# xuhuifan/FFVD

Measured on AMD Instinct MI355X. Metric: ELBO iters/sec (T=4096, M=512, x_dim=4, S=32), higher is better.
Workload: dtype f64; 1 GPU; c2: synthetic T=4096 x_dim=4 C=1 M=512 S=32 SquaredExponential collapsed-U, seed 20230209; chains_per_gpu=32, dims_per_gpu=4, arithmetic=fp64 throughout

## Files before the change

### ffvd_amd/csrc/kernels.hip

```cpp
#include "kernels.h"
#include "dev_common.h"
#define FFVD_STEP_TRACE_OWNER
#include "step_bodies.h"
#if defined(FFVD_STEP_TRACE)
extern "C" int ffvd_debug_step_spans(unsigned long long *out) {
    return (int)hipMemcpyFromSymbol(out, HIP_SYMBOL(ffvd::step_span), sizeof(unsigned long long) * 64 * 4 * 2);
}
extern "C" int ffvd_debug_step_trace(long long *out) {
    return (int)hipMemcpyFromSymbol(out, HIP_SYMBOL(ffvd::step_trace_buf), sizeof(long long) * 4096 * 8);
}
#endif
#include <type_traits>
#include <cstdlib>

namespace ffvd {

__device__ __forceinline__ double block_sum_256(double v, double *scratch ) {
    const int tid = threadIdx.x;
    scratch[tid] = v;
    __syncthreads();
    for (int s = 128; s > 0; s >>= 1) {
        if (tid < s) scratch[tid] += scratch[tid + s];
        __syncthreads();
    }
// ... 182 lines not shown
                        const double *log_Q, double yn_over_batch, double *H, size_t h_stride, int brow) {
    hipLaunchKernelGGL(brow_finish_kernel, dim3((Mp + 255) / 256, nb), dim3(256), 0, stream, gpart, nblk, Mp, Dl, d_begin, b0, log_Q,
                       yn_over_batch, H, h_stride, brow);
}
template <bool NT>
static void launch_kfu_build_nt(hipStream_t stream, const ProjectArgs &a) {
    dim3 grid(a.Tp / 64, a.Mp / 64, a.nb);
    if (a.P <= 8) {
        const int nq = (a.P + 1) / 2;
        if (a.kind == 0) {
            if (nq <= 2) hipLaunchKernelGGL((kfu_build_kernel<0, 2, NT>), grid, dim3(256), 0, stream, a);
            else if (nq == 3) hipLaunchKernelGGL((kfu_build_kernel<0, 3, NT>), grid, dim3(256), 0, stream, a);
            else hipLaunchKernelGGL((kfu_build_kernel<0, 4, NT>), grid, dim3(256), 0, stream, a);
        } else hipLaunchKernelGGL((kfu_build_kernel<1, 4, NT>), grid, dim3(256), 0, stream, a);
    } else {
        if (a.kind == 0) hipLaunchKernelGGL((kfu_build_kernel<0, 0, NT>), grid, dim3(256), 0, stream, a);
        else hipLaunchKernelGGL((kfu_build_kernel<1, 0, NT>), grid, dim3(256), 0, stream, a);
    }
}
template <int KIND, int NQ, int MW>
__global__ __launch_bounds__(256) void kfu_build_t_kernel(ProjectArgs a, int ldt) {
    kfu_build_t_body<KIND, NQ, MW>(a, ldt, blockIdx.x, blockIdx.y, blockIdx.z);
}
void launch_kfu_build_t(hipStream_t stream, const ProjectArgs &a, int ldt) {
    constexpr int MW = 4;
    dim3 grid(a.Tp / 64, a.Mp / (4 * MW), a.nb);
    if (a.P <= 8) {
        const int nq = (a.P + 1) / 2;
        if (a.kind == 0) {
            if (nq <= 2) hipLaunchKernelGGL((kfu_build_t_kernel<0, 2, MW>), grid, dim3(256), 0, stream, a, ldt);
            else if (nq == 3) hipLaunchKernelGGL((kfu_build_t_kernel<0, 3, MW>), grid, dim3(256), 0, stream, a, ldt);
            else hipLaunchKernelGGL((kfu_build_t_kernel<0, 4, MW>), grid, dim3(256), 0, stream, a, ldt);
        } else hipLaunchKernelGGL((kfu_build_t_kernel<1, 4, MW>), grid, dim3(256), 0, stream, a, ldt);
    } else {
        if (a.kind == 0) hipLaunchKernelGGL((kfu_build_t_kernel<0, 0, MW>), grid, dim3(256), 0, stream, a, ldt);
        else hipLaunchKernelGGL((kfu_build_t_kernel<1, 0, MW>), grid, dim3(256), 0, stream, a, ldt);
    }
}
void launch_kfu_build(hipStream_t stream, const ProjectArgs &a) {
    const bool nt = (size_t)a.nb * a.Tp * a.Mp * sizeof(double) >= ((size_t)1 << 30);
    if (nt) launch_kfu_build_nt<true>(stream, a);
    else launch_kfu_build_nt<false>(stream, a);
}

__global__ __launch_bounds__(256) void kernel_matrix_kernel(int kind, const double *X, int N, const double *X2, int N2,
                                                            int P, double logvar, const double *loglen, double jitter,
                                                            int same, double *out) {
    const size_t idx = (size_t)blockIdx.x * 256 + threadIdx.x;
    if (idx >= (size_t)N * N2) return;
    const int i = (int)(idx / N2), j = (int)(idx % N2);
    const double var = exp(logvar);
    const double *xi = X + (size_t)i * P, *zj = X2 + (size_t)j * P;
    double v;
    if (kind == 0) {
        double dot = 0.0, xx = 0.0, zz = 0.0;
        for (int p = 0; p < P; ++p) {
            double l = exp(loglen[p]);
            double a = xi[p] / l, b = zj[p] / l;
            dot += a * b; xx += a * a; zz += b * b;
        }
        v = kernel_value<0>(dot, xx, zz, var);
    } else {
        double dot = 0.0;
        for (int p = 0; p < P; ++p) dot += (xi[p] * var) * zj[p];
        v = dot;
    }
    if (same && i == j) v += jitter;
    out[idx] = v;
}
void launch_kernel_matrix(hipStream_t stream, int kind, const double *X, int N, const double *X2, int N2, int P,
                          double logvar, const double *loglen_dev, double jitter, int same, double *out) {
    size_t n = (size_t)N * N2;
    if (n == 0) return;
    hipLaunchKernelGGL(kernel_matrix_kernel, dim3((unsigned)((n + 255) / 256)), dim3(256), 0, stream, kind, X, N, X2,
                       N2, P, logvar, loglen_dev, jitter, same, out);
}
__global__ void kernel_diag_kernel(int kind, const double *X, int N, int P, double logvar, double *out) {
    int i = blockIdx.x * blockDim.x + threadIdx.x;
    if (i >= N) return;
    const double var = exp(logvar);
    if (kind == 0) { out[i] = var; return; }
    double s = 0.0;
    for (int p = 0; p < P; ++p) { double x = X[(size_t)i * P + p]; s += (x * x) * var; }
    out[i] = s;
}
void launch_kernel_diag(hipStream_t stream, int kind, const double *X, int N, int P, double logvar, double *out) {
    if (N == 0) return;
    hipLaunchKernelGGL(kernel_diag_kernel, dim3((N + 255) / 256), dim3(256), 0, stream, kind, X, N, P, logvar, out);
}

#ifdef FFVD_DF_TRACE
__device__ long long df_trace_buf[64 * 64];
__device__ long long gram_trace_buf[128 * 10 * 4];
#endif

constexpr int LR_LD = NB + 2;
constexpr int DV_LD = 17;
template <bool PIPE>
__device__ __forceinline__ int chol64_1w(double (&a)[NB], double (*Lr)[LR_LD], double *invd, const int lane) {
    int bad = 0;
    if (!PIPE) {
#pragma unroll
        for (int j = 0; j < NB; ++j) {
            double s0 = a[j], s1 = 0.0;
            if (j >= 2) wave_lds_sync();
#pragma unroll
            for (int i = 0; i + 1 < j - 1 + (j & 1); i += 2) {
                const double2 lj = *reinterpret_cast<const double2 *>(&Lr[j][i]);
                s0 -= a[i] * lj.x;
                s1 -= a[i + 1] * lj.y;
            }
            if (j >= 2 && !(j & 1)) s0 -= a[j - 2] * Lr[j][j - 2];
            if (j >= 1) s1 -= a[j - 1] * readlane_f64(a[j - 1], j);
            const double v = s0 + s1;
            const double ajj = readlane_f64(v, j);
            if (!(ajj > 0.0) && bad == 0) bad = j + 1;
            double piv, y;
            pivot_sqrt(ajj, piv, y);
            a[j] = v * y;
            Lr[lane][j] = a[j];
            if (lane == 0) invd[j] = y;
        }
        return bad;
    }
    double nxt = 0.0;
#pragma unroll
    for (int j = 0; j < NB; ++j) {
        double v = a[j] - nxt;
        if (j >= 2) v -= a[j - 2] * readlane_f64(a[j - 2], j);
        if (j >= 1) v -= a[j - 1] * readlane_f64(a[j - 1], j);
        const double ajj = readlane_f64(v, j);
        if (!(ajj > 0.0) && bad == 0) bad = j + 1;
        double piv, y;
        pivot_sqrt(ajj, piv, y);
        if (j + 1 < NB) {
            if (j >= 2) wave_lds_sync();
            double q0 = 0.0, q1 = 0.0, q2 = 0.0, q3 = 0.0;
#pragma unroll
            for (int i = 0; i + 1 <= j - 2; i += 2) {
                const double2 l2 = *reinterpret_cast<const double2 *>(&Lr[j + 1][i]);
                if (i & 2) { q2 += a[i] * l2.x; q3 += a[i + 1] * l2.y; }
                else { q0 += a[i] * l2.x; q1 += a[i + 1] * l2.y; }
            }
            if (j >= 2 && !(j & 1)) q0 += a[j - 2] * Lr[j + 1][j - 2];
            nxt = (q0 + q1) + (q2 + q3);
        }
        a[j] = v * y;
        Lr[lane][j] = a[j];
        if (lane == 0) invd[j] = y;
    }
    return bad;
}

__device__ __forceinline__ int chol64_mfma_4w(double (*Ts)[NB + 1], double (*Lr)[LR_LD], double (*Sc)[16][DV_LD], double *dinv_b) {
    const int lane = threadIdx.x & 63, lr = lane & 15, lk = lane >> 4;
    const int wave = __builtin_amdgcn_readfirstlane((int)(threadIdx.x >> 6));
    if (threadIdx.x < 256) Sc[3][threadIdx.x >> 4][threadIdx.x & 15] = ((threadIdx.x >> 4) == (threadIdx.x & 15)) ? 1.0 : 0.0;
    __syncthreads();
    int bad = 0;
#pragma unroll
    for (int s = 0; s < 4; ++s) {
        const int s0 = 16 * s;
        if (s > 0) {
            const int i = s + wave;
            if (i < 4) {
                const int i0 = 16 * i;
                d4 acc = (d4){0.0, 0.0, 0.0, 0.0}, acc1 = acc;
                for (int k = 0; k < s; ++k)
#pragma unroll
                    for (int t = 0; t < 4; ++t) {
                        const double av = Lr[i0 + lr][16 * k + 4 * t + lk], bv = Lr[s0 + lr][16 * k + 4 * t + lk];
                        if (t & 1) acc1 = mfma_f64(av, bv, acc1);
                        else acc = mfma_f64(av, bv, acc);
                    }
#pragma unroll
                for (int r = 0; r < 4; ++r) Sc[wave][lk + 4 * r][lr] = Ts[i0 + lk + 4 * r][s0 + lr] - (acc[r] + acc1[r]);
            }
            __syncthreads();
        }
        if (wave == 0 || (s == 0 && wave == 1)) {
            __builtin_amdgcn_s_setprio(3);
            int tl;
            if (wave == 0) tl = (lk == 0) ? 0 : (lk == 1) ? -1 : ((s + lk - 1 < 4) ? lk - 1 : -2);
            else tl = (lk == 1) ? 3 : -2;
            const double *src;
            if (tl == -1) src = &Sc[3][lr][0];
            else if (s == 0) src = &Ts[16 * (tl > 0 ? tl : 0) + lr][0];
            else src = &Sc[tl > 0 ? tl : 0][lr][0];
            double a[16];
#pragma unroll
            for (int c = 0; c < 16; ++c) a[c] = src[c];
#pragma unroll
            for (int j = 0; j < 16; ++j) {
                const double ajj = readlane_f64(a[j], j);
                double piv, y;
                pivot_sqrt(ajj, piv, y);
                a[j] *= y;
#pragma unroll
                for (int c = j + 1; c < 16; ++c) a[c] = fma(-a[j], readlane_f64(a[j], c), a[c]);
            }
            double diag = a[0];
#pragma unroll
            for (int c = 1; c < 16; ++c) diag = (lr == c) ? a[c] : diag;
            if (tl >= 0) {
                double *base = &Lr[s0 + 16 * tl + lr][s0];
#pragma unroll
                for (int c = 0; c < 16; ++c) base[c] = (tl > 0 || c <= lr) ? a[c] : 0.0;
            } else if (tl == -1) {
#pragma unroll
                for (int c = 0; c < 16; ++c) dinv_b[(s0 + c) * 16 + lr] = a[c];
            }
            if (wave == 0) {
                const unsigned long long m = __ballot((lane < 16) & !(diag > 0.0));
                if (m && !bad) bad = s0 + (int)__builtin_ctzll(m) + 1;
            }
            __builtin_amdgcn_s_setprio(0);
        }
        __syncthreads();
    }
    return bad;
}

template <bool PIPE>
__device__ __forceinline__ void diag_block_finish(double (*Ts)[NB + 1], double (*Lr)[LR_LD], double *invd, double *S, int n,
                                                   int k0, int32_t *info_b, double *dinv_b, double (*Sc)[16][DV_LD] = nullptr) {
    const int tid = threadIdx.x, lane = tid & 63;
    const int w = __builtin_amdgcn_readfirstlane(tid >> 6);
    if (Sc) {
        const int bad = chol64_mfma_4w(Ts, Lr, Sc, dinv_b);
        if (w == 0 && bad && lane == 0 && *info_b == 0) *info_b = k0 + bad;
        for (int r = tid >> 6; r < NB; r += 4)
            if (lane <= r) S[(size_t)(k0 + r) * n + k0 + lane] = Lr[r][lane];
        return;
    }
    if (w == 0) {
        double a[NB];
#pragma unroll
        for (int c = 0; c < NB; ++c) a[c] = Ts[lane][c];
        __builtin_amdgcn_s_setprio(3);
        const int bad = chol64_1w<PIPE>(a, Lr, invd, lane);
        __builtin_amdgcn_s_setprio(0);
        if (bad && lane == 0 && *info_b == 0) *info_b = k0 + bad;
    }
    __syncthreads();
    for (int r = tid >> 6; r < NB; r += 4)
        if (lane <= r) S[(size_t)(k0 + r) * n + k0 + lane] = Lr[r][lane];
    if (lane < 16) {
        const int o = 16 * w;
        double x[16];
#pragma unroll
        for (int r = 0; r < 16; ++r) {
            double acc = (lane == r) ? 1.0 : 0.0;
#pragma unroll
            for (int i = 0; i < r; ++i) acc -= Lr[o + r][o + i] * x[i];
            x[r] = acc * invd[o + r];
        }
#pragma unroll
        for (int r = 0; r < 16; ++r) dinv_b[(w * 16 + r) * 16 + lane] = x[r];
    }
}

__global__ __launch_bounds__(256) void potrf_diag_kernel(double *A, int n, int k, size_t slab_stride, int32_t *info,
                                                         double *dinv) {
    __shared__ double Ts[NB][NB + 1];
    __shared__ double Lr[NB][LR_LD];
    __shared__ double invd[NB];
    const int b = blockIdx.x, tid = threadIdx.x;
    double *S = A + (size_t)b * slab_stride;
    const int k0 = k * NB;
    for (int r = tid >> 6; r < NB; r += 4) Ts[r][tid & 63] = S[(size_t)(k0 + r) * n + k0 + (tid & 63)];
    __syncthreads();
    diag_block_finish<true>(Ts, Lr, invd, S, n, k0, info + b, dinv + (size_t)b * DINV_STRIDE);
}

__device__ __forceinline__ int extra_block(int e, int nlive, int nid) { return (e < nlive) ? e : nid + (e - nlive); }
__device__ __forceinline__ int chunk_row0(int chunk, int k, int nmain, int n, int nlive, int nid) {
    return (chunk < nmain) ? (k + 1 + chunk) * NB : n + extra_block(chunk - nmain, nlive, nid) * NB;
}

constexpr int TR_LD = NB + 2;

__global__ __launch_bounds__(256) void potrf_panel_kernel(double *A, int n, int k, int nmain, size_t slab_stride,
                                                          int nlive, int nid, const double *dinv) {
    __shared__ double Ls[NB][TR_LD];
    __shared__ double Dv[4][16][DV_LD];
    const int b = blockIdx.y, tid = threadIdx.x, lane = tid & 63, lr = lane & 15, lk = lane >> 4;
    const int w = __builtin_amdgcn_readfirstlane(tid >> 6);
    double *S = A + (size_t)b * slab_stride;
    const int k0 = k * NB;
    const int row0 = chunk_row0(blockIdx.x, k, nmain, n, nlive, nid);
    double *Rl = S + (size_t)(row0 + 16 * w + lr) * n + k0 + lk;
    d4 Rt[4];
#pragma unroll
    for (int s4 = 0; s4 < 4; ++s4)
#pragma unroll
        for (int r = 0; r < 4; ++r) Rt[s4][r] = Rl[16 * s4 + 4 * r];
#pragma unroll
    for (int i = 0; i < 8; ++i) {
        const int r = (tid >> 5) + 8 * i, c2 = 2 * (tid & 31);
        const double2 v = *reinterpret_cast<const double2 *>(S + (size_t)(k0 + r) * n + k0 + c2);
        Ls[r][c2] = (c2 <= r) ? -v.x : 0.0;
        Ls[r][c2 + 1] = (c2 + 1 <= r) ? -v.y : 0.0;
    }
    {
        const double *dv = dinv + (size_t)b * DINV_STRIDE;
#pragma unroll
        for (int i = 0; i < 4; ++i) {
            const int e = tid + 256 * i;
            Dv[e >> 8][(e >> 4) & 15][e & 15] = dv[e];
        }
    }
    __syncthreads();
#pragma unroll
    for (int s4 = 0; s4 < 4; ++s4) {
        d4 x = (d4){0.0, 0.0, 0.0, 0.0};
#pragma unroll
        for (int ks = 0; ks < 4; ++ks) x = mfma_f64(Dv[s4][lr][4 * ks + lk], Rt[s4][ks], x);
        d4 res = Rt[s4];
#pragma unroll
        for (int ks = 0; ks < 4; ++ks) res = mfma_f64(Ls[16 * s4 + lr][16 * s4 + 4 * ks + lk], x[ks], res);
#pragma unroll
        for (int ks = 0; ks < 4; ++ks) x = mfma_f64(Dv[s4][lr][4 * ks + lk], res[ks], x);
        Rt[s4] = x;
#pragma unroll
        for (int t = s4 + 1; t < 4; ++t)
#pragma unroll
            for (int ks = 0; ks < 4; ++ks) Rt[t] = mfma_f64(Ls[16 * t + lr][16 * s4 + 4 * ks + lk], x[ks], Rt[t]);
    }
#pragma unroll
    for (int s4 = 0; s4 < 4; ++s4)
#pragma unroll
        for (int r = 0; r < 4; ++r) Rl[16 * s4 + 4 * r] = Rt[s4][r];
}

template <bool PIPE>
__global__ __launch_bounds__(256) void potrf_trail_kernel(double *A, int n, int k, int nmain_tiles, int n1,
                                                          size_t slab_stride, int32_t *info, int nlive, int nid,
                                                          double *dinv) {
    constexpr int HLD = 34;
    __shared__ double sm[2 * NB * HLD];
    __shared__ double invd[NB];
    static_assert(2 * NB * HLD >= NB * LR_LD, "the staging buffer must hold the factor tile");
    double *Pi_h = sm, *Pj_h = sm + NB * HLD;
    const int b = blockIdx.y;
    const int tile = blockIdx.x;
    double *S = A + (size_t)b * slab_stride;
    const int k0 = k * NB;
    int rowblk0, colblk;
    if (tile < nmain_tiles) {
        int i = 0;
        while ((i + 1) * (i + 2) / 2 <= tile) ++i;
        int j = tile - i * (i + 1) / 2;
        rowblk0 = (k + 1 + i) * NB;
        colblk = (k + 1 + j) * NB;
    } else {
        int t = tile - nmain_tiles;
        int e = t / n1, j = t % n1;
        rowblk0 = n + extra_block(e, nlive, nid) * NB;
        colblk = (k + 1 + j) * NB;
    }
    const int tid = threadIdx.x, lane = tid & 63, lr = lane & 15, lk = lane >> 4;
    const int wave = __builtin_amdgcn_readfirstlane(tid >> 6);
    const int qr = wave >> 1, qc = wave & 1;
    const bool same = (rowblk0 == colblk);
    const double *Pi = S + (size_t)rowblk0 * n + k0;
    const double *Pj = S + (size_t)colblk * n + k0;
    const int sr = tid >> 4, sc = 2 * (tid & 15);
    double2 vi[2][4], vj[2][4];
#pragma unroll
    for (int h = 0; h < 2; ++h)
#pragma unroll
        for (int i = 0; i < 4; ++i) {
            vi[h][i] = *reinterpret_cast<const double2 *>(Pi + (size_t)(sr + 16 * i) * n + 32 * h + sc);
            if (!same) vj[h][i] = *reinterpret_cast<const double2 *>(Pj + (size_t)(sr + 16 * i) * n + 32 * h + sc);
        }
    const double *Bh = same ? Pi_h : Pj_h;
    double *Ct = S + (size_t)rowblk0 * n + colblk;
    d4 cold[2][2];
#pragma unroll
    for (int x = 0; x < 2; ++x)
#pragma unroll
        for (int y = 0; y < 2; ++y)
#pragma unroll
            for (int q = 0; q < 4; ++q)
                cold[x][y][q] = Ct[(size_t)(qr * 32 + 16 * x + lk + 4 * q) * n + qc * 32 + 16 * y + lr];
// ... 171 lines not shown
#pragma unroll
    for (int s4 = 0; s4 < 4; ++s4) {
        d4 x = (d4){0.0, 0.0, 0.0, 0.0};
#pragma unroll
        for (int ks = 0; ks < 4; ++ks) x = mfma_f64(Dv[s4][lr][4 * ks + lk], Rt[s4][ks], x);
        d4 res = Rt[s4];
#pragma unroll
        for (int ks = 0; ks < 4; ++ks) res = mfma_f64(Ls[16 * s4 + lr][16 * s4 + 4 * ks + lk], x[ks], res);
#pragma unroll
        for (int ks = 0; ks < 4; ++ks) x = mfma_f64(Dv[s4][lr][4 * ks + lk], res[ks], x);
        Rt[s4] = x;
#pragma unroll
        for (int t = s4 + 1; t < 4; ++t)
#pragma unroll
            for (int ks = 0; ks < 4; ++ks) Rt[t] = mfma_f64(Ls[16 * t + lr][16 * s4 + 4 * ks + lk], x[ks], Rt[t]);
    }
    double *Rl = S + (size_t)(row0 + 16 * wave + lr) * n + j0 + lk;
#pragma unroll
    for (int s4 = 0; s4 < 4; ++s4)
#pragma unroll
        for (int r = 0; r < 4; ++r) Rl[16 * s4 + 4 * r] = Rt[s4][r];
    if (!look) return;
#pragma unroll
    for (int s4 = 0; s4 < 4; ++s4)
#pragma unroll
        for (int r = 0; r < 4; ++r) Xs[16 * wave + lr][16 * s4 + 4 * r + lk] = Rt[s4][r];
    __syncthreads();
    if (do_d) {
#pragma unroll 4
        for (int ks = 0; ks < NB / 4; ++ks) {
            double ax[2], bx[2];
#pragma unroll
            for (int x = 0; x < 2; ++x) {
                ax[x] = Xs[qr * 32 + 16 * x + lr][4 * ks + lk];
                bx[x] = Xs[qc * 32 + 16 * x + lr][4 * ks + lk];
            }
#pragma unroll
            for (int x = 0; x < 2; ++x)
#pragma unroll
                for (int y = 0; y < 2; ++y) acc_d[x][y] = mfma_f64(ax[x], bx[y], acc_d[x][y]);
        }
    }
    double (*Ts)[NB + 1] = reinterpret_cast<double(*)[NB + 1]>(sm1);
    double (*Lr)[LR_LD] = reinterpret_cast<double(*)[LR_LD]>(sm1);
#pragma unroll
    for (int x = 0; x < 2; ++x)
#pragma unroll
        for (int y = 0; y < 2; ++y)
#pragma unroll
            for (int q = 0; q < 4; ++q)
                Ts[qr * 32 + 16 * x + lk + 4 * q][qc * 32 + 16 * y + lr] = cold_d[x][y][q] - acc_d[x][y][q];
    __syncthreads();
    diag_block_finish<PIPE>(Ts, Lr, invd, S, n, j0 + NB, info + b, dinv + (size_t)b * DINV_STRIDE + ((j + 1) & 1) * (DINV_STRIDE / 2));
}

__global__ __launch_bounds__(256) void diag_inv_kernel(const double *A, int n, int j, size_t slab_stride, double *dinv) {
    __shared__ double Lr[NB][NB + 1];
    const int b = blockIdx.x, tid = threadIdx.x, lane = tid & 63;
    const int w = __builtin_amdgcn_readfirstlane(tid >> 6);
    const double *S = A + (size_t)b * slab_stride;
    const int j0 = j * NB;
    for (int r = tid >> 6; r < NB; r += 4) Lr[r][lane] = S[(size_t)(j0 + r) * n + j0 + lane];
    __syncthreads();
    if (lane < 16) {
        const int o = 16 * w;
        double x[16];
#pragma unroll
        for (int r = 0; r < 16; ++r) {
            double acc = (lane == r) ? 1.0 : 0.0;
#pragma unroll
            for (int i = 0; i < r; ++i) acc -= Lr[o + r][o + i] * x[i];
            x[r] = acc / Lr[o + r][o + r];
        }
        double *dv = dinv + (size_t)b * DINV_STRIDE + (j & 1) * (DINV_STRIDE / 2);
#pragma unroll
        for (int r = 0; r < 16; ++r) dv[(w * 16 + r) * 16 + lane] = x[r];
    }
}

void launch_trsm_ext(hipStream_t stream, double *A, int n, int extra_rows, int batch, size_t slab_stride, double *dinv) {
    const int nb = n / NB, ntail = extra_rows / NB;
    if (ntail == 0) return;
    const int groups = (batch + 7) / 8;
    for (int j = 0; j < nb; ++j) {
        hipLaunchKernelGGL(diag_inv_kernel, dim3(batch), dim3(256), 0, stream, A, n, j, slab_stride, dinv);
        hipLaunchKernelGGL(potrf_ll_kernel<false>, dim3(groups * 8 * ntail), dim3(256), 0, stream, A, n, j, 0, ntail,
                           slab_stride, (int32_t *)nullptr, 0, 0, batch, dinv);
    }
}

constexpr int DF_PS = 64;
static_assert(DF_PS == 64, "launch_kuu_build zeroes 64 progress words per matrix");
constexpr int DF_DINV = 4 * 16 * 16;
constexpr long long DF_SPIN_TICKS = 100000000LL;

struct DfArgs {
    double *A;
    int n, nb, next, nid, batch, G;
    size_t slab_stride;
    int32_t *info;
    double *dinv;
    int *prog;
    int *abort_w;
    double *xt;
    size_t xt_stride;
    int vec_tail;
    double *kinv;
    size_t kinv_stride;
    int defer_ext;
    int kinv_help;
    int fine;
    const double *lt;
    size_t lt_stride;
    int lt_dl;
};

#ifdef FFVD_DF_TRACE
#define DF_STAMP(row, slot) do { if ((row) >= 0 && threadIdx.x == 0) df_trace_buf[(row) * 64 + (slot)] = wall_clock64(); } while (0)
extern "C" int ffvd_debug_df_trace(long long *out) {
    return (int)hipMemcpyFromSymbol(out, HIP_SYMBOL(df_trace_buf), sizeof(long long) * 64 * 64);
}
extern "C" int ffvd_debug_gram_trace(long long *out) {
    return (int)hipMemcpyFromSymbol(out, HIP_SYMBOL(gram_trace_buf), sizeof(long long) * 128 * 10 * 4);
}
#else
#define DF_STAMP(row, slot) do { } while (0)
#endif

__device__ __forceinline__ int df_wait(int *flag, int need, int *abort_w, int *slot) {
    if (threadIdx.x == 0) {
        int v = __hip_atomic_load(flag, __ATOMIC_RELAXED, __HIP_MEMORY_SCOPE_AGENT);
        if (v < need) {
            const long long t0 = wall_clock64();
            for (;;) {
                __builtin_amdgcn_s_sleep(2);
                v = __hip_atomic_load(flag, __ATOMIC_RELAXED, __HIP_MEMORY_SCOPE_AGENT);
                if (v >= need) break;
                if (__hip_atomic_load(abort_w, __ATOMIC_RELAXED, __HIP_MEMORY_SCOPE_AGENT) != 0) { v = -1; break; }
                if (wall_clock64() - t0 > DF_SPIN_TICKS) {
                    __hip_atomic_store(abort_w, 1, __ATOMIC_RELAXED, __HIP_MEMORY_SCOPE_AGENT);
                    v = -1;
                    break;
                }
            }
        }
        __builtin_amdgcn_fence(__ATOMIC_ACQUIRE, "agent");
        asm volatile("s_waitcnt vmcnt(0)" ::: "memory");
        *slot = v;
    }
    __syncthreads();
    return *slot;
}

__device__ __forceinline__ void df_publish(int *flag, int value) {
    __builtin_amdgcn_fence(__ATOMIC_RELEASE, "agent");
    asm volatile("s_waitcnt vmcnt(0)" ::: "memory");
    __hip_atomic_store(flag, value, __ATOMIC_RELAXED, __HIP_MEMORY_SCOPE_AGENT);
    asm volatile("s_waitcnt vmcnt(0)" ::: "memory");
}

template <bool LAST, bool EARLY = false>
__device__ __forceinline__ bool df_column(const DfArgs &a, double *S, int *pg, const double *dvb, const int row0, const int j,
                                          const int k0, double (*Xs)[LL_LD], double (*Ls)[LL_LD], double (*Dv)[16][DV_LD],
                                          int *wslot, int &wc, d4 (&cold_d)[2][2], d4 (&acc_d)[2][2], const int trow,
                                          double *xt_row = nullptr, const double *lt_src = nullptr, const int lt_e = 0) {
    const int n = a.n;
    DF_STAMP(trow, 5 * (j & 7) + 0);
    const int tid = threadIdx.x, lane = tid & 63, lr = lane & 15, lk = lane >> 4;
    const int wave = __builtin_amdgcn_readfirstlane(tid >> 6);
    const int qr = wave >> 1, qc = wave & 1;
    const int sr = tid >> 5, sc = 2 * (tid & 31);
    const int j0 = j * NB;
    const bool tri = !(qr == 0 && qc == 1);
    const bool do_d = LAST && tri && a.fine != 1;
    d4 cold_t[2][2], acc_t[2][2];
#pragma unroll
    for (int x = 0; x < 2; ++x)
#pragma unroll
        for (int y = 0; y < 2; ++y) {
#pragma unroll
            for (int q = 0; q < 4; ++q) {
                const size_t rr = (size_t)(row0 + qr * 32 + 16 * x + lk + 4 * q), cc = (size_t)(qc * 32 + 16 * y + lr);
                if (!LAST && lt_src) {
                    const int il = qr * 32 + 16 * x + lk + 4 * q, cl = (int)cc;
                    const double v = lt_src[(size_t)(j0 + cl) * n + lt_e * NB + il];
                    cold_t[x][y][q] = (j > lt_e || cl >= il) ? v : 0.0;
                } else cold_t[x][y][q] = S[rr * n + j0 + cc];
                if (LAST) cold_d[x][y][q] = S[rr * n + row0 + cc];
            }
            acc_t[x][y] = (d4){0.0, 0.0, 0.0, 0.0};
        }
    int seen = -2;
    if (j > k0) {
        int *pc = pg + 2 * a.nb + j;
        int have = 0;
        if (a.fine) {
            have = df_wait(pc, k0 + 1, a.abort_w, &wslot[wc++ & 1]);
            if (have < 0) return false;
        } else {
            seen = df_wait(pg + j, j, a.abort_w, &wslot[wc++ & 1]);
            if (seen < 0) return false;
        }
        DF_STAMP(trow, 5 * (j & 7) + 1);
        d2 vx[8], vl[8];
        auto gload = [&](int k) {
#pragma unroll
            for (int i = 0; i < 8; ++i) {
                vl[i] = *reinterpret_cast<const d2 *>(S + (size_t)(j0 + sr + 8 * i) * n + k * NB + sc);
                vx[i] = *reinterpret_cast<const d2 *>(S + (size_t)(row0 + sr + 8 * i) * n + k * NB + sc);
            }
        };
        gload(k0);
        for (int k = k0; k < j; ++k) {
            if (k > k0) __syncthreads();
#pragma unroll
            for (int i = 0; i < 8; ++i) {
                Ls[sr + 8 * i][sc] = vl[i].x; Ls[sr + 8 * i][sc + 1] = vl[i].y;
                Xs[sr + 8 * i][sc] = vx[i].x; Xs[sr + 8 * i][sc + 1] = vx[i].y;
            }
            __syncthreads();
            if (k + 1 < j) {
                if (a.fine && have < k + 2) {
                    have = df_wait(pc, k + 2, a.abort_w, &wslot[wc++ & 1]);
                    if (have < 0) return false;
                }
                gload(k + 1);
            }
#pragma unroll 4
            for (int ks = 0; ks < NB / 4; ++ks) {
                double bl[2], ax[2], bx[2];
#pragma unroll
                for (int x = 0; x < 2; ++x) {
                    bl[x] = Ls[qc * 32 + 16 * x + lr][4 * ks + lk];
                    ax[x] = Xs[qr * 32 + 16 * x + lr][4 * ks + lk];
                    bx[x] = do_d ? Xs[qc * 32 + 16 * x + lr][4 * ks + lk] : 0.0;
                }
#pragma unroll
                for (int x = 0; x < 2; ++x)
#pragma unroll
                    for (int y = 0; y < 2; ++y) acc_t[x][y] = mfma_f64(ax[x], bl[y], acc_t[x][y]);
                if (do_d) {
#pragma unroll
                    for (int x = 0; x < 2; ++x)
#pragma unroll
                        for (int y = 0; y < 2; ++y) acc_d[x][y] = mfma_f64(ax[x], bx[y], acc_d[x][y]);
                }
            }
        }
        __syncthreads();
    }
    DF_STAMP(trow, 5 * (j & 7) + 2);
#pragma unroll
    for (int x = 0; x < 2; ++x)
#pragma unroll
        for (int y = 0; y < 2; ++y)
#pragma unroll
            for (int q = 0; q < 4; ++q)
                Xs[qr * 32 + 16 * x + lk + 4 * q][qc * 32 + 16 * y + lr] = cold_t[x][y][q] - acc_t[x][y][q];
    if (seen < j + 1) {
        seen = df_wait(pg + j, j + 1, a.abort_w, &wslot[wc++ & 1]);
        if (seen < 0) return false;
    }
    DF_STAMP(trow, 5 * (j & 7) + 3);
#pragma unroll
    for (int i = 0; i < 8; ++i) {
        const int r = sr + 8 * i;
        const d2 v = *reinterpret_cast<const d2 *>(S + (size_t)(j0 + r) * n + j0 + sc);
        Ls[r][sc] = (sc <= r) ? -v.x : 0.0;
        Ls[r][sc + 1] = (sc + 1 <= r) ? -v.y : 0.0;
    }
    {
        const double *dv = dvb + (size_t)j * DF_DINV;
#pragma unroll
        for (int i = 0; i < 4; ++i) {
            const int e = tid + 256 * i;
            Dv[e >> 8][(e >> 4) & 15][e & 15] = dv[e];
        }
    }
    __syncthreads();
    DF_STAMP(trow, 52 + (j & 7));
    d4 Rt[4];
#pragma unroll
    for (int s4 = 0; s4 < 4; ++s4)
#pragma unroll
        for (int r = 0; r < 4; ++r) Rt[s4][r] = Xs[16 * wave + lr][16 * s4 + 4 * r + lk];
#pragma unroll
    for (int s4 = 0; s4 < 4; ++s4) {
        d4 x = (d4){0.0, 0.0, 0.0, 0.0};
#pragma unroll
        for (int ks = 0; ks < 4; ++ks) x = mfma_f64(Dv[s4][lr][4 * ks + lk], Rt[s4][ks], x);
        d4 res = Rt[s4];
#pragma unroll
        for (int ks = 0; ks < 4; ++ks) res = mfma_f64(Ls[16 * s4 + lr][16 * s4 + 4 * ks + lk], x[ks], res);
#pragma unroll
        for (int ks = 0; ks < 4; ++ks) x = mfma_f64(Dv[s4][lr][4 * ks + lk], res[ks], x);
        Rt[s4] = x;
#pragma unroll
        for (int t = s4 + 1; t < 4; ++t)
#pragma unroll
            for (int ks = 0; ks < 4; ++ks) Rt[t] = mfma_f64(Ls[16 * t + lr][16 * s4 + 4 * ks + lk], x[ks], Rt[t]);
    }
    double *Rl = S + (size_t)(row0 + 16 * wave + lr) * n + j0 + lk;
#pragma unroll
    for (int s4 = 0; s4 < 4; ++s4)
#pragma unroll
        for (int r = 0; r < 4; ++r) Rl[16 * s4 + 4 * r] = Rt[s4][r];
    if (!LAST && xt_row) {
        double *Tl = xt_row + (size_t)(j0 + lk) * n + 16 * wave + lr;
#pragma unroll
        for (int s4 = 0; s4 < 4; ++s4)
#pragma unroll
            for (int r = 0; r < 4; ++r) Tl[(size_t)(16 * s4 + 4 * r) * n] = Rt[s4][r];
    }
    if (LAST) {
#pragma unroll
        for (int s4 = 0; s4 < 4; ++s4)
#pragma unroll
            for (int r = 0; r < 4; ++r) Xs[16 * wave + lr][16 * s4 + 4 * r + lk] = Rt[s4][r];
        asm volatile("s_waitcnt lgkmcnt(0)\n\ts_barrier" ::: "memory");
    } else if (EARLY) {
#pragma unroll
        for (int s4 = 0; s4 < 4; ++s4)
#pragma unroll
            for (int r = 0; r < 4; ++r) Xs[16 * wave + lr][16 * s4 + 4 * r + lk] = Rt[s4][r];
        asm volatile("s_waitcnt vmcnt(0) lgkmcnt(0)" ::: "memory");
        __syncthreads();
        if (tid == 64) df_publish(pg + 2 * a.nb + row0 / NB, j + 1);
        if (tri) {
#pragma unroll 4
            for (int ks = 0; ks < NB / 4; ++ks) {
                double ax[2], bx[2];
#pragma unroll
                for (int x = 0; x < 2; ++x) {
                    ax[x] = Xs[qr * 32 + 16 * x + lr][4 * ks + lk];
                    bx[x] = Xs[qc * 32 + 16 * x + lr][4 * ks + lk];
                }
#pragma unroll
                for (int x = 0; x < 2; ++x)
#pragma unroll
                    for (int y = 0; y < 2; ++y) acc_d[x][y] = mfma_f64(ax[x], bx[y], acc_d[x][y]);
            }
        }
        __syncthreads();
    } else {
        if (a.fine && row0 < n) {
            asm volatile("s_waitcnt vmcnt(0)" ::: "memory");
            __syncthreads();
            if (tid == 64) df_publish(pg + 2 * a.nb + row0 / NB, j + 1);
        } else __syncthreads();
    }
    DF_STAMP(trow, 5 * (j & 7) + 4);
    return true;
}

__device__ __forceinline__ void df_vector_row(const DfArgs &a, double *S, int *pg, const double *dvb, const int row0, const int b,
                                              double *xv , double (*Ls)[LL_LD], double *part ,
                                              double *invd , int *wslot) {
    const int n = a.n, nb = a.nb, tid = threadIdx.x, c = tid & 63;
    const int q = __builtin_amdgcn_readfirstlane(tid >> 6);
    const int sr = tid >> 5, sc = 2 * (tid & 31);
    double *v = S + (size_t)row0 * n;
    int wc = 0;
    for (int j = 0; j < nb; ++j) {
        const int j0 = j * NB;
        const double vj = v[j0 + c];
        double acc = 0.0;
        int seen = -2;
        if (j > 0) {
            seen = df_wait(pg + j, j, a.abort_w, &wslot[wc++ & 1]);
            if (seen < 0) { if (tid == 0 && a.info) a.info[b] = -1; return; }
            const double *Lrow = S + (size_t)(j0 + c) * n + 16 * q;
            for (int k = 0; k < j; ++k) {
                const double *xp = xv + k * NB + 16 * q;
#pragma unroll
                for (int m = 0; m < 16; m += 2) {
                    const d2 l = *reinterpret_cast<const d2 *>(Lrow + k * NB + m);
                    acc = fma(xp[m], l.x, acc);
                    acc = fma(xp[m + 1], l.y, acc);
                }
            }
        }
        part[q * 64 + c] = acc;
        if (seen < j + 1) {
            seen = df_wait(pg + j, j + 1, a.abort_w, &wslot[wc++ & 1]);
            if (seen < 0) { if (tid == 0 && a.info) a.info[b] = -1; return; }
        } else __syncthreads();
#pragma unroll
        for (int i = 0; i < 8; ++i) {
            const int r = sr + 8 * i;
            const d2 l = *reinterpret_cast<const d2 *>(S + (size_t)(j0 + r) * n + j0 + sc);
            Ls[r][sc] = l.x; Ls[r][sc + 1] = l.y;
        }
        if (tid < 64) invd[tid] = dvb[(size_t)j * DF_DINV + ((tid >> 4) * 16 + (tid & 15)) * 16 + (tid & 15)];
        __syncthreads();
        if (q == 0) {
            double t = vj - ((part[c] + part[64 + c]) + (part[128 + c] + part[192 + c]));
            double x = 0.0;
#pragma unroll
            for (int m = 0; m < NB; ++m) {
                const double xm = readlane_f64(t, m) * invd[m];
                if (c == m) x = xm;
                if (c > m) t = fma(-xm, Ls[c][m], t);
            }
            v[j0 + c] = x;
            xv[j0 + c] = x;
        }
        __syncthreads();
    }
}

__device__ __forceinline__ bool df_inverse_tiles(const DfArgs &a, double *S, int *pg, const int b, const int e,
                                                 double (*Xs)[LL_LD], double (*Ls)[LL_LD], int *wslot, const bool helper = false) {
    const int n = a.n, nb = a.nb;
    const int tid = threadIdx.x, lane = tid & 63, lr = lane & 15, lk = lane >> 4;
    const int wave = __builtin_amdgcn_readfirstlane(tid >> 6);
    const int qr = wave >> 1, qc = wave & 1;
    const int sr = tid >> 5, sc = 2 * (tid & 31);
    int wc = 0;
    if (!helper) {
        asm volatile("s_waitcnt vmcnt(0)" ::: "memory");
        __syncthreads();
        if (tid == 0) df_publish(pg + nb + e, 1);
    } else if (e > 0) {
        const int seen = df_wait(pg + nb + e, 1, a.abort_w, &wslot[wc++ & 1]);
        if (seen < 0) return false;
    }
    double *Kb = a.kinv + (size_t)b * a.kinv_stride;
    const double *We = S + (size_t)(n + e * NB) * n;
    for (int f = 0; f <= e; ++f) {
        if (a.kinv_help && (((e + f) & 1) != 0) != helper) continue;
        if (f < e) {
            const int seen = df_wait(pg + nb + f, 1, a.abort_w, &wslot[wc++ & 1]);
            if (seen < 0) return false;
        }
        const double *Wf = S + (size_t)(n + f * NB) * n;
        d4 acc[2][2];
#pragma unroll
        for (int x = 0; x < 2; ++x)
#pragma unroll
            for (int y = 0; y < 2; ++y) acc[x][y] = (d4){0.0, 0.0, 0.0, 0.0};
        d2 vx[8], vl[8];
        auto gload = [&](int j) {
#pragma unroll
            for (int i = 0; i < 8; ++i) {
                vx[i] = *reinterpret_cast<const d2 *>(We + (size_t)(sr + 8 * i) * n + j * NB + sc);
                vl[i] = *reinterpret_cast<const d2 *>(Wf + (size_t)(sr + 8 * i) * n + j * NB + sc);
            }
        };
        gload(e);
        for (int j = e; j < nb; ++j) {
            __syncthreads();
#pragma unroll
            for (int i = 0; i < 8; ++i) {
                Xs[sr + 8 * i][sc] = vx[i].x; Xs[sr + 8 * i][sc + 1] = vx[i].y;
                Ls[sr + 8 * i][sc] = vl[i].x; Ls[sr + 8 * i][sc + 1] = vl[i].y;
            }
            __syncthreads();
            if (j + 1 < nb) gload(j + 1);
#pragma unroll 4
            for (int ks = 0; ks < NB / 4; ++ks) {
                double ax[2], bl[2];
#pragma unroll
                for (int x = 0; x < 2; ++x) {
                    ax[x] = Xs[qr * 32 + 16 * x + lr][4 * ks + lk];
                    bl[x] = Ls[qc * 32 + 16 * x + lr][4 * ks + lk];
                }
#pragma unroll
                for (int x = 0; x < 2; ++x)
#pragma unroll
                    for (int y = 0; y < 2; ++y) acc[x][y] = mfma_f64(ax[x], bl[y], acc[x][y]);
            }
        }
#pragma unroll
        for (int x = 0; x < 2; ++x)
#pragma unroll
            for (int y = 0; y < 2; ++y)
#pragma unroll
                for (int q = 0; q < 4; ++q) {
                    const size_t i = (size_t)(e * NB + qr * 32 + 16 * x + lk + 4 * q), jj = (size_t)(f * NB + qc * 32 + 16 * y + lr);
                    Kb[i * n + jj] = acc[x][y][q];
                    if (f < e) Kb[jj * n + i] = acc[x][y][q];
                }
    }
    return true;
}

template <bool PIPE>
__global__ __launch_bounds__(256, 2) void potrf_df_kernel(DfArgs a) {
    __shared__ double sm0[NB * LL_LD];
    __shared__ double sm1[NB * LL_LD];
    __shared__ double invd[NB];
    __shared__ double Dv[4][16][DV_LD];
    __shared__ int wslot[2];
    const int n = a.n, nb = a.nb;
    int grp, rem, ri;
    if (a.defer_ext) {
        const int rows_a = nb + a.next - a.nid, per_a = rows_a * a.G, n_a = ((a.batch + a.G - 1) / a.G) * per_a;
        if ((int)blockIdx.x < n_a) {
            grp = blockIdx.x / per_a; rem = blockIdx.x % per_a;
            const int rr = rem / a.G;
            ri = (rr < nb) ? rr : rr + a.nid;
        } else {
            const int id2 = blockIdx.x - n_a, per_b = a.nid * a.G;
            grp = id2 / per_b; rem = id2 % per_b;
            ri = nb + rem / a.G;
        }
    } else {
        const int per_group = (nb + a.next) * a.G;
        grp = blockIdx.x / per_group; rem = blockIdx.x % per_group;
        ri = rem / a.G;
    }
    const int b = grp * a.G + rem % a.G;
    if (b >= a.batch) return;
    const int tid = threadIdx.x, lane = tid & 63, lr = lane & 15, lk = lane >> 4;
    const int wave = __builtin_amdgcn_readfirstlane(tid >> 6);
    const int qr = wave >> 1, qc = wave & 1;
    double *S = a.A + (size_t)b * a.slab_stride;
    int *pg = a.prog + (size_t)b * DF_PS;
    double *dvb = a.dinv + (size_t)b * nb * DF_DINV;
    const bool main_row = ri < nb;
    int row0, k0 = 0, ncols;
    if (main_row) { row0 = ri * NB; ncols = ri; }
    else {
        const int e = ri - nb;
        row0 = n + e * NB; ncols = nb;
        if (e < a.nid) k0 = e;
    }
    double (*Xs)[LL_LD] = reinterpret_cast<double(*)[LL_LD]>(sm0);
    double (*Ls)[LL_LD] = reinterpret_cast<double(*)[LL_LD]>(sm1);
    if (!main_row && a.vec_tail && ri - nb >= a.nid) {
        df_vector_row(a, S, pg, dvb, row0, b, sm0, Ls, &Dv[0][0][0], invd, wslot);
        return;
    }
    int wc = 0;
    const int trow = (b == 0) ? ri : -1;
    DF_STAMP(trow, 51);
    d4 cold_d[2][2], acc_d[2][2];
#pragma unroll
    for (int x = 0; x < 2; ++x)
#pragma unroll
        for (int y = 0; y < 2; ++y) acc_d[x][y] = (d4){0.0, 0.0, 0.0, 0.0};
    {
        const int nplain = main_row ? ncols - 1 : ncols;
        double *xt_row = (a.xt && !main_row && ri - nb < a.nid) ? a.xt + (size_t)b * a.xt_stride + (size_t)(ri - nb) * NB : nullptr;
        const double *lt_src = (a.lt && !main_row && ri - nb < a.nid) ? a.lt + (size_t)(b % a.lt_dl) * a.lt_stride : nullptr;
        if (main_row && a.fine == 1) {
            for (int j = 0; j < nplain; ++j) {
                if (!df_column<false, true>(a, S, pg, dvb, row0, j, 0, Xs, Ls, Dv, wslot, wc, cold_d, acc_d, trow)) {
                    if (tid == 0 && a.info) a.info[b] = -1;
                    return;
                }
            }
        } else {
            for (int j = k0; j < nplain; ++j) {
                d4 unused_c[2][2], unused_a[2][2];
                if (!df_column<false>(a, S, pg, dvb, row0, j, k0, Xs, Ls, Dv, wslot, wc, unused_c, unused_a, trow, xt_row, lt_src,
                                      ri - nb)) {
                    if (tid == 0 && a.info) a.info[b] = -1;
                    return;
                }
            }
        }
    }
    if (!main_row) {
        if (a.kinv && ri - nb < a.nid && !df_inverse_tiles(a, S, pg, b, ri - nb, Xs, Ls, wslot)) {
            if (tid == 0 && a.info) a.info[b] = -1;
        }
        return;
    }
    if (ncols > 0) {
        if (!df_column<true>(a, S, pg, dvb, row0, ncols - 1, k0, Xs, Ls, Dv, wslot, wc, cold_d, acc_d, trow)) {
            if (tid == 0 && a.info) a.info[b] = -1;
            return;
        }
        if (!(qr == 0 && qc == 1)) {
#pragma unroll 4
            for (int ks = 0; ks < NB / 4; ++ks) {
                double ax[2], bx[2];
#pragma unroll
                for (int x = 0; x < 2; ++x) {
                    ax[x] = Xs[qr * 32 + 16 * x + lr][4 * ks + lk];
                    bx[x] = Xs[qc * 32 + 16 * x + lr][4 * ks + lk];
                }
#pragma unroll
                for (int x = 0; x < 2; ++x)
#pragma unroll
                    for (int y = 0; y < 2; ++y) acc_d[x][y] = mfma_f64(ax[x], bx[y], acc_d[x][y]);
            }
        }
    } else {
#pragma unroll
        for (int x = 0; x < 2; ++x)
#pragma unroll
            for (int y = 0; y < 2; ++y)
#pragma unroll
                for (int q = 0; q < 4; ++q)
                    cold_d[x][y][q] = S[(size_t)(row0 + qr * 32 + 16 * x + lk + 4 * q) * n + row0 + qc * 32 + 16 * y + lr];
    }
    double (*Ts)[NB + 1] = reinterpret_cast<double(*)[NB + 1]>(sm1);
#pragma unroll
    for (int x = 0; x < 2; ++x)
#pragma unroll
        for (int y = 0; y < 2; ++y)
#pragma unroll
            for (int q = 0; q < 4; ++q)
                Ts[qr * 32 + 16 * x + lk + 4 * q][qc * 32 + 16 * y + lr] = cold_d[x][y][q] - acc_d[x][y][q];
    asm volatile("s_waitcnt vmcnt(0)" ::: "memory");
    __syncthreads();
    double (*Lr)[LR_LD] = reinterpret_cast<double(*)[LR_LD]>(sm0);
    DF_STAMP(trow, 48);
    if (ncols > 0 && tid == 64) {
        df_publish(pg + ri, ri);
        if (a.fine) __hip_atomic_store(pg + 2 * nb + ri, ri, __ATOMIC_RELAXED, __HIP_MEMORY_SCOPE_AGENT);
    }
    diag_block_finish<PIPE>(Ts, Lr, invd, S, n, row0, a.info + b, dvb + (size_t)ri * DF_DINV, Dv);
    asm volatile("s_waitcnt vmcnt(0)" ::: "memory");
    __syncthreads();
    DF_STAMP(trow, 49);
#ifdef FFVD_DF_TEST_STALL
    if (b == 0 && ri == 0) return;
#endif
    if (tid == 0) df_publish(pg + ri, ri + 1);
    DF_STAMP(trow, 50);
    if (a.kinv_help) {
        __syncthreads();
        if (!df_inverse_tiles(a, S, pg, b, ri, Xs, Ls, wslot, true)) {
            if (tid == 0 && a.info) a.info[b] = -1;
        }
    }
}

size_t potrf_scratch_doubles(int n, int batch) {
    const size_t nb = (size_t)(n / NB), bt = (size_t)(batch > 0 ? batch : 1);
    const size_t flow = ((bt * DF_PS + 4) * sizeof(int) + 15) / 16 * 2 + bt * nb * DF_DINV;
    const size_t step = bt * DINV_STRIDE;
    return flow > step ? flow : step;
}

void potrf_flow_clear(hipStream_t stream, double *scratch, int batch) {
    const size_t words = ((size_t)batch * DF_PS + 4 + 3) / 4 * 4;
    const size_t n = words / 2;
    hipLaunchKernelGGL(fill_kernel, dim3((unsigned)((n + 255) / 256)), dim3(256), 0, stream, scratch, n, 0.0);
}

static void launch_potrf_flow(hipStream_t stream, double *A, int n, int extra_rows, int identity_rows, int batch,
                              size_t slab_stride, int32_t *info, double *scratch, double *linv_t, size_t linv_t_stride,
                              bool words_zeroed, bool tail_is_vector, double *kinv, size_t kinv_stride, const double *lt_rows,
                              size_t lt_stride, int lt_dl, bool kinv_help) {
    DfArgs a{};
    a.lt = lt_rows; a.lt_stride = lt_stride; a.lt_dl = lt_dl > 0 ? lt_dl : 1;
    a.xt = linv_t; a.xt_stride = linv_t_stride;
    a.vec_tail = tail_is_vector ? 1 : 0;
    if (kinv && identity_rows == n && 2 * (n / NB) <= DF_PS) { a.kinv = kinv; a.kinv_stride = kinv_stride; }
    a.A = A; a.n = n; a.nb = n / NB; a.next = extra_rows / NB; a.nid = identity_rows / NB; a.batch = batch;
    a.slab_stride = slab_stride; a.info = info;
    const size_t words = ((size_t)batch * DF_PS + 4 + 3) / 4 * 4;
    a.prog = reinterpret_cast<int *>(scratch);
    a.abort_w = a.prog + (size_t)batch * DF_PS;
    a.dinv = scratch + words / 2;
    if (!words_zeroed) potrf_flow_clear(stream, scratch, batch);
    const int R = a.nb + a.next, bp = (batch + 7) / 8 * 8;
    a.G = ((size_t)bp * R <= 2048) ? bp : ((1024 / R + 7) / 8 * 8 < 8 ? 8 : (1024 / R + 7) / 8 * 8);
    if (a.G > bp) a.G = bp;
    const int groups = (batch + a.G - 1) / a.G;
    static const int defer_mode = [] { const char *e = getenv("FFVD_DF_DEFER"); return e ? atoi(e) : -1; }();
    a.defer_ext = (a.nid > 0 && groups > 1 && !a.xt && !a.kinv && defer_mode != 0) ? 1 : 0;
    const bool one_per_cu = (size_t)batch * R <= 256 || (a.nid == 0 && (size_t)batch * R <= 640);
    a.kinv_help = (kinv_help && a.kinv && a.nid == a.nb && (size_t)batch * R <= 256) ? 1 : 0;
    const bool alone = one_per_cu;
    const int fine_mode = [] { const char *e = getenv("FFVD_DF_FINE"); return e ? atoi(e) : -1; }();
    a.fine = ((fine_mode >= 0 ? fine_mode != 0 : (alone && (size_t)batch * R <= 256)) && 3 * a.nb <= DF_PS) ? (fine_mode == 2 ? 2 : 1) : 0;
    hipLaunchKernelGGL(potrf_df_kernel<true>, dim3((unsigned)((size_t)groups * R * a.G)), dim3(256), alone ? 16384 : 0, stream, a);
}

static int chol_mode() {
    static const int v = [] {
        const char *e = getenv("FFVD_CHOL");
        if (!e) return 0;
        return (e[0] == 'l') ? 1 : ((e[0] == 'r') ? 2 : ((e[0] == 'f') ? 3 : 0));
    }();
    return v;
}
static thread_local int g_chol_override = 0;
void potrf_override_variant(int variant) { g_chol_override = variant; }
int potrf_override_current() { return g_chol_override; }
static int chol_variant(int batch, int nb, int hint);
bool potrf_flow_selected(int n, int batch, int hint) { return chol_variant(batch, n / NB, hint) == 3; }
bool potrf_flow_forms_inverse(int n, int batch, int hint) { return potrf_flow_selected(n, batch, hint) && 2 * (n / NB) <= DF_PS; }
static int chol_variant(int batch, int nb, int hint) {
    int m = g_chol_override ? g_chol_override : chol_mode();
    if (m == 0) m = (hint == CHOL_FLOW || batch >= 32) ? 3 : 2;
    if (m == 3 && nb > DF_PS) m = 1;
    return m;
}

void launch_potrf_ext(hipStream_t stream, double *A, int n, int extra_rows, int identity_rows, int batch,
                      size_t slab_stride, int32_t *info, double *dinv, int hint, double *linv_t, size_t linv_t_stride,
                      bool words_zeroed, bool tail_is_vector, double *kinv, size_t kinv_stride, const double *lt_rows,
                      size_t lt_stride, int lt_dl, bool kinv_help) {
    const int nb = n / NB;
    const int nid = identity_rows / NB, ntail = extra_rows / NB - nid;
    const int variant = chol_variant(batch, nb, hint);
    if (variant == 3) {
        launch_potrf_flow(stream, A, n, extra_rows, identity_rows, batch, slab_stride, info, dinv, linv_t, linv_t_stride, words_zeroed,
                          tail_is_vector, kinv, kinv_stride, lt_rows, lt_stride, lt_dl, kinv_help);
        return;
    }
    if (variant == 1) {
        const int groups = (batch + 7) / 8;
        hipLaunchKernelGGL(potrf_diag_kernel, dim3(batch), dim3(256), 0, stream, A, n, 0, slab_stride, info, dinv);
        for (int j = 0; j < nb; ++j) {
            const int nmain = nb - j - 1;
            const int nlive = (j + 1 < nid) ? j + 1 : nid;
            const int nchunks = nmain + nlive + ntail;
            if (nchunks == 0) continue;
            if ((size_t)nchunks * batch <= 512)
                hipLaunchKernelGGL(potrf_ll_kernel<true>, dim3(groups * 8 * nchunks), dim3(256), 0, stream, A, n, j, nmain,
                                   nchunks, slab_stride, info, nlive, nid, batch, dinv);
            else
                hipLaunchKernelGGL(potrf_ll_kernel<false>, dim3(groups * 8 * nchunks), dim3(256), 0, stream, A, n, j, nmain,
                                   nchunks, slab_stride, info, nlive, nid, batch, dinv);
        }
        return;
    }
// ... 1266 lines not shown
```

Before: 322.5 iters/sec.

## Use sc1 write-through stores for hand-off tiles and drop publish fences

Tiles produced in the dataflow Cholesky and consumed by other blocks are now written with sc1 write-through vector stores (dwordx4) or agent-scope atomic stores, staged through LDS so rows go out coalesced. The release fence and vmcnt waits in df_publish are removed, on the assumption that the write-through stores are already globally visible once counted. This is meant to cut the cache-writeback cost of agent-scope release fences on every inter-block hand-off. It ties correctness to gfx942/gfx950 store semantics, enforced with a compile-time error on other targets, and risks memory-ordering races if the assumption fails.

```diff
diff --git a/ffvd_amd/csrc/kernels.hip b/ffvd_amd/csrc/kernels.hip
--- a/ffvd_amd/csrc/kernels.hip
+++ b/ffvd_amd/csrc/kernels.hip
@@ -358,6 +358,17 @@
     return bad;
 }
 
+#if defined(__HIP_DEVICE_COMPILE__) && !defined(__gfx950__) && !defined(__gfx942__)
+#error "potrf_df_kernel's hand-offs rely on gfx942/gfx950 store semantics (vmcnt-counted sc1 write-through stores); build for gfx950"
+#endif
+__device__ __forceinline__ void df_store_wt16(double *p, const d2 v) {
+    asm volatile("global_store_dwordx4 %0, %1, off sc1" : : "v"(p), "v"(v) : "memory");
+}
+__device__ __forceinline__ void df_store_wt8(double *p, const double v) {
+    typedef __attribute__((address_space(1))) double gdouble;
+    __hip_atomic_store((gdouble *)p, v, __ATOMIC_RELAXED, __HIP_MEMORY_SCOPE_AGENT);
+}
+
 __device__ __forceinline__ int chol64_mfma_4w(double (*Ts)[NB + 1], double (*Lr)[LR_LD], double (*Sc)[16][DV_LD], double *dinv_b) {
     const int lane = threadIdx.x & 63, lr = lane & 15, lk = lane >> 4;
     const int wave = __builtin_amdgcn_readfirstlane((int)(threadIdx.x >> 6));
@@ -414,7 +425,7 @@
                 for (int c = 0; c < 16; ++c) base[c] = (tl > 0 || c <= lr) ? a[c] : 0.0;
             } else if (tl == -1) {
 #pragma unroll
-                for (int c = 0; c < 16; ++c) dinv_b[(s0 + c) * 16 + lr] = a[c];
+                for (int c = 0; c < 16; ++c) df_store_wt8(dinv_b + (s0 + c) * 16 + lr, a[c]);
             }
             if (wave == 0) {
                 const unsigned long long m = __ballot((lane < 16) & !(diag > 0.0));
@@ -435,8 +446,14 @@
     if (Sc) {
         const int bad = chol64_mfma_4w(Ts, Lr, Sc, dinv_b);
         if (w == 0 && bad && lane == 0 && *info_b == 0) *info_b = k0 + bad;
-        for (int r = tid >> 6; r < NB; r += 4)
-            if (lane <= r) S[(size_t)(k0 + r) * n + k0 + lane] = Lr[r][lane];
+        const int c = 2 * (tid & 31);
+#pragma unroll
+        for (int i = 0; i < 8; ++i) {
+            const int r = (tid >> 5) + 8 * i;
+            double *p = S + (size_t)(k0 + r) * n + k0 + c;
+            if (c + 1 <= r) df_store_wt16(p, *reinterpret_cast<const d2 *>(&Lr[r][c]));
+            else if (c == r) df_store_wt8(p, Lr[r][c]);
+        }
         return;
     }
     if (w == 0) {
@@ -914,18 +931,27 @@
     return *slot;
 }
 
+__device__ __forceinline__ void df_store_tile_rows(double *dst , const int n,
+                                                   const double (*T)[LL_LD] , const int lane, const bool wt) {
+    const int r = lane >> 5, c = 2 * (lane & 31);
+#pragma unroll
+    for (int i = 0; i < 8; ++i) {
+        const d2 v = *reinterpret_cast<const d2 *>(&T[2 * i + r][c]);
+        double *p = dst + (size_t)(2 * i + r) * n + c;
+        if (wt) df_store_wt16(p, v);
+        else *reinterpret_cast<d2 *>(p) = v;
+    }
+}
+
 __device__ __forceinline__ void df_publish(int *flag, int value) {
-    __builtin_amdgcn_fence(__ATOMIC_RELEASE, "agent");
-    asm volatile("s_waitcnt vmcnt(0)" ::: "memory");
     __hip_atomic_store(flag, value, __ATOMIC_RELAXED, __HIP_MEMORY_SCOPE_AGENT);
-    asm volatile("s_waitcnt vmcnt(0)" ::: "memory");
 }
 
 template <bool LAST, bool EARLY = false>
 __device__ __forceinline__ bool df_column(const DfArgs &a, double *S, int *pg, const double *dvb, const int row0, const int j,
                                           const int k0, double (*Xs)[LL_LD], double (*Ls)[LL_LD], double (*Dv)[16][DV_LD],
                                           int *wslot, int &wc, d4 (&cold_d)[2][2], d4 (&acc_d)[2][2], const int trow,
-                                          double *xt_row = nullptr, const double *lt_src = nullptr, const int lt_e = 0) {
+                                          const bool wt, double *xt_row = nullptr, const double *lt_src = nullptr, const int lt_e = 0) {
     const int n = a.n;
     DF_STAMP(trow, 5 * (j & 7) + 0);
     const int tid = threadIdx.x, lane = tid & 63, lr = lane & 15, lk = lane >> 4;
@@ -1062,11 +1088,11 @@
 #pragma unroll
             for (int ks = 0; ks < 4; ++ks) Rt[t] = mfma_f64(Ls[16 * t + lr][16 * s4 + 4 * ks + lk], x[ks], Rt[t]);
     }
-    double *Rl = S + (size_t)(row0 + 16 * wave + lr) * n + j0 + lk;
 #pragma unroll
     for (int s4 = 0; s4 < 4; ++s4)
 #pragma unroll
-        for (int r = 0; r < 4; ++r) Rl[16 * s4 + 4 * r] = Rt[s4][r];
+        for (int r = 0; r < 4; ++r) Xs[16 * wave + lr][16 * s4 + 4 * r + lk] = Rt[s4][r];
+    df_store_tile_rows(S + (size_t)(row0 + 16 * wave) * n + j0, n, Xs + 16 * wave, lane, wt);
     if (!LAST && xt_row) {
         double *Tl = xt_row + (size_t)(j0 + lk) * n + 16 * wave + lr;
 #pragma unroll
@@ -1075,16 +1101,8 @@
             for (int r = 0; r < 4; ++r) Tl[(size_t)(16 * s4 + 4 * r) * n] = Rt[s4][r];
     }
     if (LAST) {
-#pragma unroll
-        for (int s4 = 0; s4 < 4; ++s4)
-#pragma unroll
-            for (int r = 0; r < 4; ++r) Xs[16 * wave + lr][16 * s4 + 4 * r + lk] = Rt[s4][r];
         asm volatile("s_waitcnt lgkmcnt(0)\n\ts_barrier" ::: "memory");
     } else if (EARLY) {
-#pragma unroll
-        for (int s4 = 0; s4 < 4; ++s4)
-#pragma unroll
-            for (int r = 0; r < 4; ++r) Xs[16 * wave + lr][16 * s4 + 4 * r + lk] = Rt[s4][r];
         asm volatile("s_waitcnt vmcnt(0) lgkmcnt(0)" ::: "memory");
         __syncthreads();
         if (tid == 64) df_publish(pg + 2 * a.nb + row0 / NB, j + 1);
@@ -1249,8 +1267,8 @@
 
 template <bool PIPE>
 __global__ __launch_bounds__(256, 2) void potrf_df_kernel(DfArgs a) {
-    __shared__ double sm0[NB * LL_LD];
-    __shared__ double sm1[NB * LL_LD];
+    __shared__ __attribute__((aligned(16))) double sm0[NB * LL_LD];
+    __shared__ __attribute__((aligned(16))) double sm1[NB * LL_LD];
     __shared__ double invd[NB];
     __shared__ double Dv[4][16][DV_LD];
     __shared__ int wslot[2];
@@ -1306,9 +1324,10 @@
         const int nplain = main_row ? ncols - 1 : ncols;
         double *xt_row = (a.xt && !main_row && ri - nb < a.nid) ? a.xt + (size_t)b * a.xt_stride + (size_t)(ri - nb) * NB : nullptr;
         const double *lt_src = (a.lt && !main_row && ri - nb < a.nid) ? a.lt + (size_t)(b % a.lt_dl) * a.lt_stride : nullptr;
+        const bool wt = main_row || (a.kinv && ri - nb < a.nid);
         if (main_row && a.fine == 1) {
             for (int j = 0; j < nplain; ++j) {
-                if (!df_column<false, true>(a, S, pg, dvb, row0, j, 0, Xs, Ls, Dv, wslot, wc, cold_d, acc_d, trow)) {
+                if (!df_column<false, true>(a, S, pg, dvb, row0, j, 0, Xs, Ls, Dv, wslot, wc, cold_d, acc_d, trow, true)) {
                     if (tid == 0 && a.info) a.info[b] = -1;
                     return;
                 }
@@ -1316,7 +1335,7 @@
         } else {
             for (int j = k0; j < nplain; ++j) {
                 d4 unused_c[2][2], unused_a[2][2];
-                if (!df_column<false>(a, S, pg, dvb, row0, j, k0, Xs, Ls, Dv, wslot, wc, unused_c, unused_a, trow, xt_row, lt_src,
+                if (!df_column<false>(a, S, pg, dvb, row0, j, k0, Xs, Ls, Dv, wslot, wc, unused_c, unused_a, trow, wt, xt_row, lt_src,
                                       ri - nb)) {
                     if (tid == 0 && a.info) a.info[b] = -1;
                     return;
@@ -1331,7 +1350,7 @@
         return;
     }
     if (ncols > 0) {
-        if (!df_column<true>(a, S, pg, dvb, row0, ncols - 1, k0, Xs, Ls, Dv, wslot, wc, cold_d, acc_d, trow)) {
+        if (!df_column<true>(a, S, pg, dvb, row0, ncols - 1, k0, Xs, Ls, Dv, wslot, wc, cold_d, acc_d, trow, true)) {
             if (tid == 0 && a.info) a.info[b] = -1;
             return;
         }
```

New measurement: 322.3 iters/sec, median of 2. No clear change (-0.1%).
